# xinntao/EDVR

Measured on AMD Instinct MI355X. Metric: EDVR-L x4 5-frame 720p clips/sec, higher is better.
Workload: dtype fp32 emulated as 2xf16 (hi+lo, 22-bit operands, 4 cross products), fp32 accumulate; 1 GPU; EDVR-L x4, 5 frames, 180x320 LR -> 720x1280, batch 10/GPU, inference; clips_per_gpu=10, global_clips=10, parallelism=clip-sharded x1, no data-path collective, world_size=1, backend=single process

## Files before the change

edvr_amd/_lib.py:

```python
import ctypes
import os

_HERE = os.path.dirname(os.path.abspath(__file__))
LIB_PATH = os.environ.get('EDVR_AMD_LIB') or os.path.join(_HERE, 'lib', 'libedvr_amd.so')

c_float_p = ctypes.c_void_p
i32, i64, f32, sz = ctypes.c_int, ctypes.c_int64, ctypes.c_float, ctypes.c_size_t
vp = ctypes.c_void_p


class ConvDesc(ctypes.Structure):
    _fields_ = [
        ('x1', vp), ('x2', vp), ('c1', i32), ('c2', i32), ('x1_img_stride', i64), ('x2_img_stride', i64),
        ('x2_div', i32), ('x2_mul', i32), ('x2_add', i32), ('n', i32), ('h', i32), ('w', i32), ('wpk', vp),
        ('bias', vp), ('co', i32), ('ks', i32), ('stride', i32), ('act', i32), ('act_from', i32), ('res1', vp),
        ('res2', vp), ('res1_img_stride', i64), ('res2_img_stride', i64), ('y', vp), ('y_img_stride', i64),
        ('out_mode', i32), ('algo', i32), ('gate', vp), ('gate_img_stride', i64), ('gate_slope', f32), ('y_scale', f32),
        ('wpk_f4', vp), ('abs_sum', vp), ('abs_sum_channels', i32), ('wpk_f4s', vp), ('x_amax', vp), ('y_amax', vp),
        ('pre', vp), ('pre_img_stride', i64), ('pre_div', i32), ('pre_mul', i32), ('pre_add', i32), ('pre_n', i32), ('wpk_ds', vp),
    ]


PROTOTYPES = {
    'edvr_version': (ctypes.c_char_p, []),
# ... 14 lines not shown
    'edvr_conv2d_pack_weights_multi': (i32, [vp, i32, i32, i32, vp]),
    'edvr_conv2d_f32': (i32, [ctypes.POINTER(ConvDesc), vp]),
    'edvr_conv2d_kernel': (i32, [ctypes.POINTER(ConvDesc)]),
    'edvr_conv2d_gate_supported': (i32, [ctypes.POINTER(ConvDesc)]),
    'edvr_conv2d_abs_sum_supported': (i32, [ctypes.POINTER(ConvDesc)]),
    'edvr_conv2d_y_amax_supported': (i32, [ctypes.POINTER(ConvDesc)]),
    'edvr_conv2d_pre_supported': (i32, [ctypes.POINTER(ConvDesc)]),
    'edvr_conv2d_f4s_set_lean': (i32, [i32]),
    'edvr_conv2d_f4s_lean_items': (i32, [ctypes.POINTER(ConvDesc)]),
    'edvr_conv2d_kernel_name': (i32, [ctypes.POINTER(ConvDesc), ctypes.c_char_p, sz]),
    'edvr_conv2d_executed_flops': (i32, [ctypes.POINTER(ConvDesc), ctypes.POINTER(ctypes.c_double)]),
    'edvr_dcnv2_fwd_ws_bytes': (sz, [i32] * 12),
    'edvr_dcnv2_fwd_f32': (i32, [vp] * 6 + [i32] * 12 + [i64, i64, i32, i32, vp, sz, vp]),
    'edvr_dcnv2_fwd_split_f32': (i32, [vp] * 6 + [i32] * 12 + [i64, i64, i32, i32, vp, sz, vp, vp]),
    'edvr_dcnv2_fwd_split_applies': (i32, [vp] + [i32] * 13),
    'edvr_dcnv2_fwd_kernel_name': (i32, [vp] + [i32] * 13 + [ctypes.c_char_p, sz]),
    'edvr_dcnv2_bwd_ws_bytes': (sz, [i32] * 12),
    'edvr_dcnv2_any_ws_bytes': (sz, [i32] * 13),
    'edvr_dcnv2_fwd_any': (i32, [i32] + [vp] * 6 + [i32] * 12 + [i64, i64, vp, sz, vp]),
    'edvr_dcnv2_bwd_any': (i32, [i32] + [vp] * 10 + [i32] * 12 + [i64, i64, i64, i64, vp, sz, vp]),
    'edvr_psnr_sse_f32': (i32, [vp, vp, vp, i32, i32, i32, i32, i64, i64, i32, i32, i32, vp]),
    'edvr_ssim_partials': (sz, [i32, i32, i32]),
    'edvr_ssim_f32': (i32, [vp, vp, vp, i32, i32, i32, i32, i64, i64, i32, i32, vp]),
    'edvr_niqe_blocks': (sz, [i32, i32, i32]),
    'edvr_niqe_moments_f32': (i32, [vp, vp, i32, i32, i32, i32, i64, i32, vp]),
    'edvr_niqe_moments_u8': (i32, [vp, vp, i32, i32, i32, i64, i32, vp]),
    'edvr_frames_u8_to_f32': (i32, [vp, vp, i32, i32, i32, i32, vp, i32, vp]),
    'edvr_gather_images_f32': (i32, [vp, vp, vp, vp, i32, vp, i32, i32, vp]),
    'edvr_upsample4x_add_u8': (i32, [vp, vp, vp, i32, i32, i32, vp]),
    'edvr_f32_to_u8_hwc': (i32, [vp, vp, i32, i32, i32, i64, vp]),
# ... 109 lines not shown
```

edvr_amd/csrc/common.h:

```cpp
#pragma once
#include <hip/hip_runtime.h>

#include <cstdarg>
#include <cstdio>

#include "../../include/edvr_amd.h"

namespace edvr {

void set_error(const char *fmt, ...);

inline int check_launch(const char *what) {
  hipError_t e = hipGetLastError();
  if (e != hipSuccess) {
    set_error("%s: %s", what, hipGetErrorString(e));
    return EDVR_ERR_LAUNCH;
  }
  return EDVR_OK;
}

inline hipStream_t as_stream(edvr_stream_t s) { return reinterpret_cast<hipStream_t>(s); }

inline int cdiv(int a, int b) { return (a + b - 1) / b; }
inline int64_t cdiv64(int64_t a, int64_t b) { return (a + b - 1) / b; }
// ... 81 lines not shown
  int64_t doff_bs, dmsk_bs;
};
int dcn_fill_shape(DcnShape &s, int B, int C, int H, int W, int Co, int kh, int kw, int stride, int pad, int dil, int groups, int dg,
                   int64_t off_bs, int64_t msk_bs);

bool dcn_fused_supported(int C, int Co, int H, int W, int kh, int kw, int stride, int pad, int dil, int groups, int dg);
int dcn_fused_pack(const float *weight, float *wpk, int Co, int C, hipStream_t stream);
int dcn_fused_forward(const float *x, const float *offset, const float *mask, const float *wpk, const float *bias, float *y, int B, int C,
                      int H, int W, int Co, int dg, int64_t off_bs, int64_t msk_bs, int act, int halo, hipStream_t stream);

bool dcn_tapwin_supported(int C, int Co, int H, int W, int kh, int kw, int stride, int pad, int dil, int groups, int dg);
int dcn_tapwin_forward(const float *x, const float *offset, const float *mask, const float *wpk, const float *bias, float *y, int B, int C,
                       int H, int W, int Co, int dg, int64_t off_bs, int64_t msk_bs, int act, hipStream_t stream);

bool dcn_tapwin_split_enabled();
int dcn_tapwin_split_forward(const float *x, const float *offset, const float *mask, const float *weight, unsigned *wpk, const float *bias, float *y,
                             int B, int C, int H, int W, int Co, int dg, int64_t off_bs, int64_t msk_bs, int act, const float *xm_amax,
                             hipStream_t stream);

bool dcn_bwd_fused_supported(const DcnShape &s);
size_t dcn_bwd_fused_wbk_elems(int dg);
int dcn_bwd_fused_launch(const DcnShape &s, const float *x, const float *offset, const float *mask, const float *weight, const float *dy,
                         float *wbk, float *col, float *dx, float *doffset, float *dmask, hipStream_t stream);

__device__ inline int xcd_remap(int linear, int total) {
  const int q = total >> 3, rem = total & 7, xcd = linear & 7;
  return xcd * q + (xcd < rem ? xcd : rem) + (linear >> 3);
}
__device__ inline void xcd_block_index(int &bx, int &by, int &bz) {
  const int gx = gridDim.x, gy = gridDim.y;
// ... 17 lines not shown
```

edvr_amd/csrc/dcn.hip:

```cpp
#include <cstdlib>

#include "common.h"
#include "dcn_tap.h"

namespace edvr {

typedef float f32x16 __attribute__((ext_vector_type(16)));

__global__ void fill_kernel(float *__restrict__ p, float v, int64_t n) {
  for (int64_t i = (int64_t)blockIdx.x * blockDim.x + threadIdx.x; i < n; i += (int64_t)gridDim.x * blockDim.x) p[i] = v;
}

struct Merge {
  bool give01, give11;
  bool take00, take10;
};
__device__ __forceinline__ Merge merge_right(const Tap &t, bool same_plane_as_next) {
  Merge mg;
  const int lane = __lane_id();
  const int n_o00 = lane_next_i(t.o00), n_o10 = lane_next_i(t.o10);
  const int n_ok = lane_next_i((t.ok00 ? 1 : 0) | (t.ok10 ? 2 : 0));
  const bool has_next = lane < 63 && same_plane_as_next;
  mg.give01 = has_next && t.ok01 && (n_ok & 1) && n_o00 == t.o01;
  mg.give11 = has_next && t.ok11 && (n_ok & 2) && n_o10 == t.o11;
// ... 653 lines not shown
                             const float *xm_amax, edvr_stream_t stream) {
  EDVR_REQUIRE(xm_amax != nullptr, "dcnv2_fwd_split: null magnitude bound");
  return dcnv2_fwd_impl(x, offset, mask, weight, bias, y, B, C, H, W, Co, kh, kw, stride, pad, dil, groups, dg, offset_bstride, mask_bstride, act,
                        halo_hint, ws, ws_bytes, xm_amax, stream);
}

int edvr_dcnv2_fwd_split_applies(const float *x, int B, int C, int H, int W, int Co, int kh, int kw, int stride, int pad, int dil, int groups,
                                 int dg, int halo_hint) {
  using namespace edvr;
  DcnShape s;
  if (dcn_fill_shape(s, B, C, H, W, Co, kh, kw, stride, pad, dil, groups, dg, 0, 0)) return 0;
  return (use_fused(s) && halo_hint == EDVR_DCN_HALO_TAPWIN && dcn_tapwin_split_enabled() &&
          dcn_tapwin_supported(C, Co, H, W, kh, kw, s.stride, s.pad, s.dil, groups, dg) && (reinterpret_cast<uintptr_t>(x) & 15) == 0) ? 1 : 0;
}

int edvr_dcnv2_fwd_kernel_name(const float *x, int B, int C, int H, int W, int Co, int kh, int kw, int stride, int pad, int dil, int groups,
                               int dg, int halo_hint, char *buf, size_t buf_len) {
  using namespace edvr;
  EDVR_REQUIRE(buf && buf_len > 0, "dcnv2_fwd_kernel_name: null buffer");
  DcnShape s;
  int rc = dcn_fill_shape(s, B, C, H, W, Co, kh, kw, stride, pad, dil, groups, dg, 0, 0);
  if (rc) return rc;
  const char *name = "dcn_im2col_kernel";
  if (use_fused(s) && halo_hint >= 0) {
    const bool tapwin = halo_hint == EDVR_DCN_HALO_TAPWIN && dcn_tapwin_supported(C, Co, H, W, kh, kw, s.stride, s.pad, s.dil, groups, dg) &&
                        (reinterpret_cast<uintptr_t>(x) & 15) == 0;
    name = tapwin ? "dcn_tapwin_fwd_kernel" : "dcn_fused_fwd_kernel";
  }
  snprintf(buf, buf_len, "%s", name);
  return EDVR_OK;
// ... 179 lines not shown
```

edvr_amd/csrc/dcn_tapwin_s.hip:

```cpp
#include <type_traits>

#include "common.h"
#include <cstdlib>

#include "dcn_tap.h"
#include "pack.h"

namespace edvr {

typedef float f32x16 __attribute__((ext_vector_type(16)));
typedef float f32x4 __attribute__((ext_vector_type(4)));
typedef float f32x2 __attribute__((ext_vector_type(2)));

namespace {
constexpr int TWS_TH = 8, TWS_TW = 32, TWS_RY = 2, TWS_RX = 2;
constexpr int TWS_IH = TWS_TH + 2 * TWS_RY;
constexpr int TWS_IW = (TWS_TW + 2 * TWS_RX + 3 + 3) / 4 * 4;
constexpr int TWS_PPR = TWS_IW / 4;
constexpr int TWS_HR = TWS_IH / 2;
constexpr int TWS_HB = TWS_HR * TWS_IW;
constexpr int TWS_CHS = TWS_IH * TWS_IW;
static_assert(TWS_HR * TWS_PPR <= 64 && TWS_IH == 2 * TWS_HR && TWS_CHS % 64 == 32, "window halves must fit one wave instruction");
constexpr int TWS_MAX_DG = 8;
constexpr int TWS_OOB = (int)0x80000000;
// ... 36 lines not shown
  const uint64_t pv = reinterpret_cast<uint64_t>(ptr);
  const uint64_t pu = ((uint64_t)(uint32_t)__builtin_amdgcn_readfirstlane((int)(pv >> 32)) << 32) |
                      (uint32_t)__builtin_amdgcn_readfirstlane((int)(uint32_t)pv);
  return __builtin_amdgcn_make_buffer_rsrc(reinterpret_cast<void *>(pu), (short)0, bytes, TWS_RSRC_FLAGS);
}

static __device__ __forceinline__ void tws_split4(const float (&x)[4], unsigned (&o)[4]) {
  asm volatile(
      "v_fma_mixlo_f16 %0, %4, 1.0, 0\n\tv_fma_mixlo_f16 %1, %5, 1.0, 0\n\tv_fma_mixlo_f16 %2, %6, 1.0, 0\n\tv_fma_mixlo_f16 %3, %7, 1.0, 0\n\t"
      "v_fma_mixhi_f16 %0, %4, 1.0, -%0 op_sel_hi:[0,0,1]\n\tv_fma_mixhi_f16 %1, %5, 1.0, -%1 op_sel_hi:[0,0,1]\n\t"
      "v_fma_mixhi_f16 %2, %6, 1.0, -%2 op_sel_hi:[0,0,1]\n\tv_fma_mixhi_f16 %3, %7, 1.0, -%3 op_sel_hi:[0,0,1]"
      : "=&v"(o[0]), "=&v"(o[1]), "=&v"(o[2]), "=&v"(o[3])
      : "v"(x[0]), "v"(x[1]), "v"(x[2]), "v"(x[3]));
}

template <int MT, int CPG>
__global__ __launch_bounds__(256, 2) void dcn_tapwin_split_fwd_kernel(const DcnTapwinSArgs a) {
  constexpr int TH = TWS_TH, TW = TWS_TW, IH = TWS_IH, IW = TWS_IW, CHS = TWS_CHS, KK = 9, OOB = TWS_OOB;
  constexpr int MB = 32 * MT, NQ = CPG / 2, KG = CPG / 8;
  constexpr int XW = CPG * CHS;
  constexpr int WS = CPG * MB;
  constexpr int CPW = CPG / 4;
  static_assert(CPG % 4 == 0, "four waves share the channels of a group");
  __shared__ __attribute__((aligned(16))) float xw[2 * XW];
  __shared__ __attribute__((aligned(16))) unsigned wsl[2 * WS];
  __shared__ int shifts[TWS_MAX_DG * 18];
  __shared__ float tpl[4 * 3 * 64];

  const int tid = threadIdx.x, lane = tid & 63, half = lane >> 5, j = lane & 31;
  const int wave = __builtin_amdgcn_readfirstlane(tid >> 6);
  const unsigned amax_bits = (unsigned)__builtin_amdgcn_readfirstlane(__builtin_bit_cast(int, *a.xm_amax));
  const float s_x = __builtin_bit_cast(float, (unsigned)min(max(127 + 14 - ((int)((amax_bits >> 23) & 255u) - 127), 7), 220) << 23);
  const float unscale = (1.f / s_x) * __builtin_bit_cast(float, __builtin_amdgcn_readfirstlane((int)a.wpk[1]));
  int tile, blk_y, img;
  xcd_block_index(tile, blk_y, img);
  tile = __builtin_amdgcn_readfirstlane(tile);
  blk_y = __builtin_amdgcn_readfirstlane(blk_y);
  img = __builtin_amdgcn_readfirstlane(img);
  const int ty0 = (tile / a.tiles_x) * TH, tx0 = (tile % a.tiles_x) * TW;
  const int co_blk = a.co_start + blk_y * MB;
  const int P = a.H * a.W;
  const float *x_img = a.x + (int64_t)img * a.C * P;
  const float *off_b = a.offset + (int64_t)img * a.off_bs;
  const float *msk_b = a.mask + (int64_t)img * a.msk_bs;

  for (int v = tid; v < a.dg * 18; v += 256) {
    const float *pl = off_b + (int64_t)v * P;
    float mn = 3.0e38f, mx = -3.0e38f;
#pragma unroll
    for (int r = 1; r < TH; r += 4) {
      const int yy = min(ty0 + r, a.H - 1);
#pragma unroll
      for (int c = 4; c < TW; c += 8) {
        const float f = pl[yy * a.W + min(tx0 + c, a.W - 1)];
        mn = fminf(mn, f);
        mx = fmaxf(mx, f);
      }
    }
    const float mid = fminf(fmaxf(0.5f * (mn + mx), -16384.f), 16384.f);
    shifts[v] = (int)floorf(mid + 0.5f);
  }

  const int oy0 = ty0 + 2 * wave, ox = tx0 + j;
  const bool ok0 = oy0 < a.H && ox < a.W, ok1 = oy0 + 1 < a.H && ox < a.W;
  const int p0 = oy0 * a.W + ox;
  const int tvo[2] = {ok0 ? p0 * 4 : OOB, ok1 ? (p0 + a.W) * 4 : OOB};

  f32x16 acc[2][MT];
#pragma unroll
  for (int s = 0; s < 2; ++s)
#pragma unroll
    for (int m = 0; m < MT; ++m)
#pragma unroll
      for (int r = 0; r < 16; ++r) acc[s][m][r] = 0.f;

  const int d_r = lane / TWS_PPR, d_c = 4 * (lane - d_r * TWS_PPR);
  const int rel0 = (d_r * a.W + d_c) * 4;
  const __amdgpu_buffer_rsrc_t x_rsrc = tws_rsrc(x_img, a.C * P * 4);
  const i32x4 x_rsrc4 = tws_rsrc4(x_img, a.C * P * 4), w_rsrc4 = tws_rsrc4(a.wpk, 64 + a.C * KK * a.cop * 4);
  typedef __attribute__((address_space(3))) void lvoid;
  const unsigned xw_lds = (unsigned)(size_t)(lvoid *)xw, ws_lds = (unsigned)(size_t)(lvoid *)wsl;
  const __amdgpu_buffer_rsrc_t off_rsrc = tws_rsrc(off_b, a.dg * 18 * P * 4), msk_rsrc = tws_rsrc(msk_b, a.dg * 9 * P * 4);
  auto dma_x = [&](int buf, int g, int wy0, int wx0) {
    const int sh = (wy0 * a.W + wx0) * 4;
    const bool colok = (unsigned)(wx0 + d_c) < (unsigned)a.W;
    const int vo0 = (colok && (unsigned)(wy0 + d_r) < (unsigned)a.H) ? rel0 + sh : OOB;
    const int vo1 = (colok && (unsigned)(wy0 + d_r + TWS_HR) < (unsigned)a.H) ? rel0 + sh + TWS_HR * a.W * 4 : OOB;
    if (lane < TWS_HR * TWS_PPR) {
#pragma unroll
      for (int cc = 0; cc < CPW; ++cc) {
        const int ch = wave * CPW + cc;
        const unsigned dst = xw_lds + (buf * XW + ch * CHS) * 4;
        tws_dma16(x_rsrc4, dst, vo0, (g * CPG + ch) * P * 4);
        tws_dma16(x_rsrc4, dst + TWS_HB * 4, vo1, (g * CPG + ch) * P * 4);
      }
    }
  };
  constexpr int WTOTAL = (CPG / 4) * MB, WNI = WTOTAL / 64, WNK = (WNI + 3) / 4;
  static_assert(WTOTAL % 64 == 0, "weight slab must fill whole wave instructions");
  int wvo[WNK];
#pragma unroll
  for (int k = 0; k < WNK; ++k) {
    const int q = (wave + 4 * k) * 64 + lane, row = q / MB, c16 = q - row * MB;
    wvo[k] = (row * KK * a.cop + c16) * 16;
  }
  auto dma_w = [&](int buf, int g, int t) {
    const int so = 64 + ((g * (CPG / 4) * KK + t) * a.cop + co_blk) * 16;
#pragma unroll
    for (int k = 0; k < WNK; ++k)
      if (wave + 4 * k < WNI) tws_dma16(w_rsrc4, ws_lds + (buf * WS + (wave + 4 * k) * 256) * 4, wvo[k], so);
  };
  auto origin = [&](int g, int t, int &wy0, int &wx0) {
    const int sy = __builtin_amdgcn_readfirstlane(shifts[(g * KK + t) * 2]);
    const int sx = __builtin_amdgcn_readfirstlane(shifts[(g * KK + t) * 2 + 1]);
    const int ti = t / 3, tj = t - 3 * ti;
    wy0 = ty0 - 1 + ti + sy - TWS_RY;
    wx0 = (tx0 - 1 + tj + sx - TWS_RX) & ~3;
  };
  const i32x4 off_rsrc4 = tws_rsrc4(off_b, a.dg * 18 * P * 4), msk_rsrc4 = tws_rsrc4(msk_b, a.dg * 9 * P * 4);
  const unsigned tpl_lds = (unsigned)(size_t)(lvoid *)tpl + wave * (3 * 64 * 4);
  const int tvd = half ? tvo[1] : tvo[0];
  auto dma_taps = [&](int g, int t) {
    tws_dma4(off_rsrc4, tpl_lds, tvd, (g * 18 + 2 * t) * P * 4);
    tws_dma4(off_rsrc4, tpl_lds + 256, tvd, (g * 18 + 2 * t + 1) * P * 4);
    tws_dma4(msk_rsrc4, tpl_lds + 512, tvd, (g * 9 + t) * P * 4);
  };
  auto read_taps = [&](float (&d)[6]) {
#pragma unroll
    for (int s = 0; s < 2; ++s)
#pragma unroll
      for (int v = 0; v < 3; ++v) d[3 * s + v] = tpl[wave * 192 + v * 64 + s * 32 + j];
  };

  struct St {
    float bw[2][4];
    int addr[2];
    unsigned slow;
    unsigned slow_any;
  };
  auto state_half = [&](St &st, int s, int t, int wy0, int wx0, const float (&d)[6]) {
    const int ti = t / 3, tj = t - 3 * ti;
    const bool pix_ok = s ? ok1 : ok0;
    const float h = (float)(oy0 + s - 1 + ti) + d[3 * s], w = (float)(ox - 1 + tj) + d[3 * s + 1];
    const bool valid = pix_ok && h > -1.f && w > -1.f && h < (float)a.H && w < (float)a.W;
    const float fh = floorf(h), fw = floorf(w);
    const float lh = h - fh, lw = w - fw, m = d[3 * s + 2];
    const int ry = (int)fh - wy0, rx = (int)fw - wx0;
    const bool inside = valid && ry >= 0 && ry <= IH - 2 && rx >= 0 && rx <= IW - 2;
    const float mm = inside ? m * s_x : 0.f;
    const float hm = (1.f - lh) * mm, lm = lh * mm, hw = 1.f - lw;
    st.bw[s][0] = hm * hw;
    st.bw[s][1] = hm * lw;
    st.bw[s][2] = lm * hw;
    st.bw[s][3] = lm * lw;
    st.addr[s] = half * CHS + (inside ? ry * IW + rx : 0);
    st.slow = (s ? st.slow : 0u) | ((valid && !inside) ? 1u << s : 0u);
  };
  auto state_any = [&](St &st) { st.slow_any = __builtin_amdgcn_readfirstlane(__any(st.slow != 0) ? 1 : 0); };
  auto make_state = [&](St &st, int t, int wy0, int wx0, const float (&d)[6]) {
    state_half(st, 0, t, wy0, wx0, d);
    state_half(st, 1, t, wy0, wx0, d);
    state_any(st);
  };

  auto run_step = [&](auto SLOWT, const St &cur, const float *xb, const unsigned *wb, int g, int t, St &nxt, int tn, int ny0, int nx0,
                      const float (&tnv)[6]) {
    constexpr bool SLOW = decltype(SLOWT)::value;
    const float (&bw)[2][4] = cur.bw;
    const unsigned slow = cur.slow;
    const unsigned cbase[2] = {(unsigned)(size_t)(lvoid *)xb + (unsigned)cur.addr[0] * 4u, (unsigned)(size_t)(lvoid *)xb + (unsigned)cur.addr[1] * 4u};
    auto issue_cells = [&](int kg, float (&c)[2][4][4]) {
#pragma unroll
      for (int s = 0; s < 2; ++s) {
        typedef __attribute__((address_space(3))) const float lds_cf;
        unsigned co = cbase[s];
        asm volatile("" : "+v"(co));
#pragma unroll
        for (int i = 0; i < 4; ++i) {
          lds_cf *cell = (lds_cf *)(size_t)(co + (kg * 8 + 2 * i) * (CHS * 4));
          c[s][i][0] = cell[0];
          c[s][i][1] = cell[1];
          c[s][i][2] = cell[IW];
          c[s][i][3] = cell[IW + 1];
        }
      }
    };
    auto sample = [&](int s, const float (&c)[4]) -> float {
      return __builtin_fmaf(bw[s][3], c[3], __builtin_fmaf(bw[s][2], c[2], __builtin_fmaf(bw[s][1], c[1], bw[s][0] * c[0])));
    };
    if constexpr (SLOW) {
      const int ti = t / 3, tj = t - 3 * ti;
#pragma unroll
      for (int s = 0; s < 2; ++s) {
        if (!__any(slow >> s & 1u)) continue;
        const bool on = slow >> s & 1u;
        const int pv = on ? (p0 + s * a.W) * 4 : OOB;
        const float m = s_x * __builtin_bit_cast(float, __builtin_amdgcn_raw_buffer_load_b32(msk_rsrc, pv, (g * 9 + t) * P * 4, 0));
        const float hsp = (float)(oy0 + s - 1 + ti) + __builtin_bit_cast(float, __builtin_amdgcn_raw_buffer_load_b32(off_rsrc, pv, (g * 18 + 2 * t) * P * 4, 0));
        const float wsp = (float)(ox - 1 + tj) + __builtin_bit_cast(float, __builtin_amdgcn_raw_buffer_load_b32(off_rsrc, pv, (g * 18 + 2 * t + 1) * P * 4, 0));
        const Tap tq = resolve_tap(hsp, wsp, a.H, a.W);
        const float sw[4] = {on ? tq.w00 * m : 0.f, on ? tq.w01 * m : 0.f, on ? tq.w10 * m : 0.f, on ? tq.w11 * m : 0.f};
        const int hp = half * P;
        const int ov[4] = {on ? (tq.o00 + hp) * 4 : OOB, on ? (tq.o01 + hp) * 4 : OOB, on ? (tq.o10 + hp) * 4 : OOB, on ? (tq.o11 + hp) * 4 : OOB};
        float gv[KG][4][4];
#pragma unroll
        for (int kg = 0; kg < KG; ++kg)
#pragma unroll
          for (int i = 0; i < 4; ++i)
#pragma unroll
            for (int c = 0; c < 4; ++c)
              gv[kg][i][c] = __builtin_bit_cast(float, __builtin_amdgcn_raw_buffer_load_b32(x_rsrc, ov[c], (g * CPG + 8 * kg + 2 * i) * P * 4, 0));
#pragma unroll
        for (int kg = 0; kg < KG; ++kg) {
          i32x4 aw[MT];
#pragma unroll
          for (int m2 = 0; m2 < MT; ++m2) aw[m2] = *reinterpret_cast<const i32x4 *>(wb + ((kg * 2 + half) * MB + m2 * 32 + j) * 4);
          float v[4];
#pragma unroll
          for (int i = 0; i < 4; ++i)
            v[i] = __builtin_fmaf(sw[3], gv[kg][i][3], __builtin_fmaf(sw[2], gv[kg][i][2], __builtin_fmaf(sw[1], gv[kg][i][1], sw[0] * gv[kg][i][0])));
          unsigned pk[4];
          tws_split4(v, pk);
          i32x4 bq = i32x4{(int)pk[0], (int)pk[1], (int)pk[2], (int)pk[3]};
#pragma unroll
          for (int m2 = 0; m2 < MT; ++m2)
            acc[s][m2] = __builtin_amdgcn_mfma_f32_32x32x16_f16(__builtin_bit_cast(f16x8, aw[m2]), __builtin_bit_cast(f16x8, bq), acc[s][m2], 0, 0, 0);
          asm volatile("v_alignbit_b32 %0, %0, %0, 16\n\tv_alignbit_b32 %1, %1, %1, 16\n\tv_alignbit_b32 %2, %2, %2, 16\n\tv_alignbit_b32 %3, %3, %3, 16"
                       : "+v"(bq[0]), "+v"(bq[1]), "+v"(bq[2]), "+v"(bq[3]));
#pragma unroll
          for (int m2 = 0; m2 < MT; ++m2)
            acc[s][m2] = __builtin_amdgcn_mfma_f32_32x32x16_f16(__builtin_bit_cast(f16x8, aw[m2]), __builtin_bit_cast(f16x8, bq), acc[s][m2], 0, 0, 0);
        }
      }
    } else {
      float cv[2][4][4];
      issue_cells(0, cv);
#pragma unroll
      for (int kg = 0; kg < KG; ++kg) {
        i32x4 aw[MT];
#pragma unroll
        for (int m = 0; m < MT; ++m) aw[m] = *reinterpret_cast<const i32x4 *>(wb + ((kg * 2 + half) * MB + m * 32 + j) * 4);
        i32x4 bq[2];
#pragma unroll
        for (int s = 0; s < 2; ++s) {
          const float v[4] = {sample(s, cv[s][0]), sample(s, cv[s][1]), sample(s, cv[s][2]), sample(s, cv[s][3])};
          unsigned pk[4];
          tws_split4(v, pk);
          bq[s] = i32x4{(int)pk[0], (int)pk[1], (int)pk[2], (int)pk[3]};
        }
        if (kg + 1 < KG) issue_cells(kg + 1, cv);
#pragma unroll
        for (int s = 0; s < 2; ++s)
#pragma unroll
          for (int m = 0; m < MT; ++m)
            acc[s][m] = __builtin_amdgcn_mfma_f32_32x32x16_f16(__builtin_bit_cast(f16x8, aw[m]), __builtin_bit_cast(f16x8, bq[s]), acc[s][m], 0, 0, 0);
        if (kg == 0 || KG == 1) {
          state_half(nxt, 0, tn, ny0, nx0, tnv);
#pragma unroll
          for (int i = 0; i < 4; ++i) asm volatile("" : "+v"(nxt.bw[0][i]));
          asm volatile("" : "+v"(nxt.addr[0]), "+v"(nxt.slow));
        }
        if (kg == KG - 1) {
          state_half(nxt, 1, tn, ny0, nx0, tnv);
#pragma unroll
          for (int i = 0; i < 4; ++i) asm volatile("" : "+v"(nxt.bw[1][i]));
          asm volatile("" : "+v"(nxt.addr[1]), "+v"(nxt.slow));
          state_any(nxt);
          asm volatile("" : "+s"(nxt.slow_any));
        }
#pragma unroll
        for (int s = 0; s < 2; ++s)
          asm volatile("v_alignbit_b32 %0, %0, %0, 16\n\tv_alignbit_b32 %1, %1, %1, 16\n\tv_alignbit_b32 %2, %2, %2, 16\n\tv_alignbit_b32 %3, %3, %3, 16"
                       : "+v"(bq[s][0]), "+v"(bq[s][1]), "+v"(bq[s][2]), "+v"(bq[s][3]));
#pragma unroll
        for (int s = 0; s < 2; ++s)
#pragma unroll
          for (int m = 0; m < MT; ++m)
            acc[s][m] = __builtin_amdgcn_mfma_f32_32x32x16_f16(__builtin_bit_cast(f16x8, aw[m]), __builtin_bit_cast(f16x8, bq[s]), acc[s][m], 0, 0, 0);
        __builtin_amdgcn_sched_barrier(0);
      }
    }
  };

  __syncthreads();
  const int n_steps = a.dg * KK;
  St cur, nxt;
  float tnv[6];
  int o1y, o1x;
  origin(0, 0, o1y, o1x);
  dma_x(0, 0, o1y, o1x);
  dma_w(0, 0, 0);
  dma_taps(0, 0);
  asm volatile("s_waitcnt vmcnt(0)" ::: "memory");
  read_taps(tnv);
  make_state(cur, 0, o1y, o1x, tnv);
  asm volatile("s_waitcnt lgkmcnt(0)" ::: "memory");
  int g = 0, t = 0, g1 = 0, t1 = 1;
  if (n_steps > 1) {
    origin(g1, t1, o1y, o1x);
    dma_taps(g1, t1);
    asm volatile("s_waitcnt vmcnt(0)" ::: "memory");
  }
// ... 22 lines not shown

  const __amdgpu_buffer_rsrc_t y_rsrc = tws_rsrc(a.y + (int64_t)img * a.Co * P, a.Co * P * 4);
  const __amdgpu_buffer_rsrc_t b_rsrc = tws_rsrc(a.bias ? a.bias : a.x, a.bias ? a.Co * 4 : 0);
#pragma unroll
  for (int m = 0; m < MT; ++m) {
#pragma unroll
    for (int r4 = 0; r4 < 4; ++r4) {
      const int cob = co_blk + m * 32 + 8 * r4;
      float bias4[4];
#pragma unroll
      for (int r = 0; r < 4; ++r) {
        const bool cok = cob + 4 * half + r < a.Co;
        bias4[r] = a.bias ? __builtin_bit_cast(float, __builtin_amdgcn_raw_buffer_load_b32(b_rsrc, cok ? (4 * half + r) * 4 : OOB, cob * 4, 0)) : 0.f;
      }
#pragma unroll
      for (int s = 0; s < 2; ++s) {
        const bool pix_ok = s ? ok1 : ok0;
        const int pv = (p0 + s * a.W + 4 * half * P) * 4;
#pragma unroll
        for (int r = 0; r < 4; ++r) {
          float v = __builtin_fmaf(acc[s][m][4 * r4 + r], unscale, bias4[r]);
          if (a.act == EDVR_ACT_LRELU) v = v > 0.f ? v : 0.1f * v;
          else if (a.act == EDVR_ACT_RELU) v = fmaxf(v, 0.f);
          else if (a.act == EDVR_ACT_SIGMOID) v = __builtin_amdgcn_rcpf(1.f + __expf(-v));
          const bool cok = cob + 4 * half + r < a.Co;
          __builtin_amdgcn_raw_buffer_store_b32(__builtin_bit_cast(unsigned, v), y_rsrc, (pix_ok && cok) ? pv : OOB, (cob + r) * P * 4, 0);
        }
      }
    }
  }
}
// ... 17 lines not shown

__global__ void dcn_tapwin_split_pack_kernel(const float *__restrict__ w, unsigned *__restrict__ wpk, int Co, int C, int cop) {
  const float s_w = __builtin_bit_cast(float, wpk[0]);
  const int64_t total = (int64_t)(C / 4) * 9 * cop;
  const int full = Co / 128, rem_tiles = (Co - full * 128 + 31) / 32;
  for (int64_t i = (int64_t)blockIdx.x * blockDim.x + threadIdx.x; i < total; i += (int64_t)gridDim.x * blockDim.x) {
    const int pos = (int)(i % cop), t = (int)((i / cop) % 9), c4 = (int)(i / ((int64_t)cop * 9));
    const int blk = pos / 128 < full ? pos / 128 : full, start = blk * 128, mt = blk < full ? 4 : rem_tiles;
    const int r = pos - start, co = pos;
    const bool live = mt > 0 && r < 32 * mt && co < Co;
#pragma unroll
    for (int q = 0; q < 4; ++q) wpk[16 + i * 4 + q] = live ? split_f16x2(w[((int64_t)co * C + 8 * (c4 >> 1) + 2 * q + (c4 & 1)) * 9 + t], s_w) : 0u;
  }
}

template <int MT>
static int launch_tapwin_s(DcnTapwinSArgs a, int co_start, int co_blocks, hipStream_t stream) {
  a.co_start = co_start;
  dim3 grid(a.tiles_x * a.tiles_y, co_blocks, a.B);
  if (a.C / a.dg == 16) hipLaunchKernelGGL((dcn_tapwin_split_fwd_kernel<MT, 16>), grid, dim3(256), 0, stream, a);
  else hipLaunchKernelGGL((dcn_tapwin_split_fwd_kernel<MT, 8>), grid, dim3(256), 0, stream, a);
  return check_launch("dcn_tapwin_split_fwd_kernel");
}

bool dcn_tapwin_split_enabled() {
  static const bool on = []() {
    const char *e = getenv("EDVR_DCN_SPLIT");
    return !(e && e[0] == '0');
  }();
  return on;
}

int dcn_tapwin_split_forward(const float *x, const float *offset, const float *mask, const float *weight, unsigned *wpk, const float *bias, float *y,
                             int B, int C, int H, int W, int Co, int dg, int64_t off_bs, int64_t msk_bs, int act, const float *xm_amax,
                             hipStream_t stream) {
  EDVR_REQUIRE(B <= 65535, "dcn_tapwin_split: batch %d exceeds grid.z", B);
// ... 28 lines not shown
```

include/edvr_amd.h:

```cpp
#ifndef EDVR_AMD_H
#define EDVR_AMD_H

#include <stddef.h>
#include <stdint.h>

#ifdef __cplusplus
extern "C" {
#endif

#define EDVR_OK 0
#define EDVR_ERR_ARG (-1)
#define EDVR_ERR_UNSUPPORTED (-2)
#define EDVR_ERR_LAUNCH (-3)
#define EDVR_ERR_WORKSPACE (-4)

typedef void *edvr_stream_t;

const char *edvr_version(void);
const char *edvr_last_error(void);
int edvr_check_device(void);

#define EDVR_ACT_NONE 0
#define EDVR_ACT_RELU 1
#define EDVR_ACT_LRELU 2
// ... 87 lines not shown
#define EDVR_HW(h, w) ((int)(h) | (((int)(w) + 1) << 16))

size_t edvr_dcnv2_fwd_ws_bytes(int B, int C, int H, int W, int Co, int kh, int kw, int stride, int pad, int dil,
                               int groups, int dg);
int edvr_dcnv2_fwd_f32(const float *x, const float *offset, const float *mask, const float *weight,
                       const float *bias, float *y, int B, int C, int H, int W, int Co, int kh, int kw, int stride,
                       int pad, int dil, int groups, int dg, int64_t offset_bstride, int64_t mask_bstride, int act,
                       int halo_hint, void *ws, size_t ws_bytes, edvr_stream_t stream);

int edvr_dcnv2_fwd_split_f32(const float *x, const float *offset, const float *mask, const float *weight, const float *bias,
                             float *y, int B, int C, int H, int W, int Co, int kh, int kw, int stride, int pad, int dil, int groups,
                             int dg, int64_t offset_bstride, int64_t mask_bstride, int act, int halo_hint, void *ws, size_t ws_bytes,
                             const float *xm_amax, edvr_stream_t stream);
int edvr_dcnv2_fwd_split_applies(const float *x, int B, int C, int H, int W, int Co, int kh, int kw, int stride, int pad, int dil, int groups,
                                 int dg, int halo_hint);
int edvr_dcnv2_fwd_kernel_name(const float *x, int B, int C, int H, int W, int Co, int kh, int kw, int stride, int pad, int dil,
                               int groups, int dg, int halo_hint, char *buf, size_t buf_len);

size_t edvr_dcnv2_bwd_ws_bytes(int B, int C, int H, int W, int Co, int kh, int kw, int stride, int pad, int dil,
                               int groups, int dg);
int edvr_dcnv2_bwd_f32(const float *x, const float *offset, const float *mask, const float *weight, const float *dy,
                       float *dx, float *doffset, float *dmask, float *dweight, float *dbias, int B, int C, int H,
                       int W, int Co, int kh, int kw, int stride, int pad, int dil, int groups, int dg,
                       int64_t offset_bstride, int64_t mask_bstride, int64_t doffset_bstride, int64_t dmask_bstride,
                       int scatter_hint, void *ws, size_t ws_bytes, edvr_stream_t stream);
int edvr_dcnv2_bwd_split_f32(const float *x, const float *offset, const float *mask, const float *weight, const float *dy,
                             float *dx, float *doffset, float *dmask, float *dweight, float *dbias, int B, int C, int H,
                             int W, int Co, int kh, int kw, int stride, int pad, int dil, int groups, int dg,
                             int64_t offset_bstride, int64_t mask_bstride, int64_t doffset_bstride, int64_t dmask_bstride,
                             int scatter_hint, void *ws, size_t ws_bytes, const float *xm_amax, const float *dy_amax,
// ... 198 lines not shown
```

Baseline: 106.9 clips/s.

## Add one-row-per-wave variant of split DCN tap-window kernel with 8 waves

Templates the split-precision deformable-conv forward kernel on pixel rows per wave. The new single-row variant launches 512 threads (8 waves) and halves the per-wave accumulators and tap buffers. It is selected by default when channels per group is 16, and an env var or API call can force either mode. The aim is to cut per-wave register pressure and raise wave-level parallelism for better latency hiding. The trade-off is more waves contending for LDS and weight DMA, plus some recomputed lane offsets.

```diff
diff --git a/edvr_amd/_lib.py b/edvr_amd/_lib.py
--- a/edvr_amd/_lib.py
+++ b/edvr_amd/_lib.py
@@ -52,6 +52,7 @@
     'edvr_dcnv2_fwd_f32': (i32, [vp] * 6 + [i32] * 12 + [i64, i64, i32, i32, vp, sz, vp]),
     'edvr_dcnv2_fwd_split_f32': (i32, [vp] * 6 + [i32] * 12 + [i64, i64, i32, i32, vp, sz, vp, vp]),
     'edvr_dcnv2_fwd_split_applies': (i32, [vp] + [i32] * 13),
+    'edvr_dcnv2_fwd_split_set_rows': (i32, [i32]),
     'edvr_dcnv2_fwd_kernel_name': (i32, [vp] + [i32] * 13 + [ctypes.c_char_p, sz]),
     'edvr_dcnv2_bwd_ws_bytes': (sz, [i32] * 12),
     'edvr_dcnv2_any_ws_bytes': (sz, [i32] * 13),
diff --git a/edvr_amd/csrc/common.h b/edvr_amd/csrc/common.h
--- a/edvr_amd/csrc/common.h
+++ b/edvr_amd/csrc/common.h
@@ -119,6 +119,7 @@
                        int H, int W, int Co, int dg, int64_t off_bs, int64_t msk_bs, int act, hipStream_t stream);
 
 bool dcn_tapwin_split_enabled();
+int dcn_tapwin_split_set_rows(int rows);
 int dcn_tapwin_split_forward(const float *x, const float *offset, const float *mask, const float *weight, unsigned *wpk, const float *bias, float *y,
                              int B, int C, int H, int W, int Co, int dg, int64_t off_bs, int64_t msk_bs, int act, const float *xm_amax,
                              hipStream_t stream);
diff --git a/edvr_amd/csrc/dcn.hip b/edvr_amd/csrc/dcn.hip
--- a/edvr_amd/csrc/dcn.hip
+++ b/edvr_amd/csrc/dcn.hip
@@ -691,6 +691,8 @@
           dcn_tapwin_supported(C, Co, H, W, kh, kw, s.stride, s.pad, s.dil, groups, dg) && (reinterpret_cast<uintptr_t>(x) & 15) == 0) ? 1 : 0;
 }
 
+int edvr_dcnv2_fwd_split_set_rows(int rows) { return edvr::dcn_tapwin_split_set_rows(rows); }
+
 int edvr_dcnv2_fwd_kernel_name(const float *x, int B, int C, int H, int W, int Co, int kh, int kw, int stride, int pad, int dil, int groups,
                                int dg, int halo_hint, char *buf, size_t buf_len) {
   using namespace edvr;
diff --git a/edvr_amd/csrc/dcn_tapwin_s.hip b/edvr_amd/csrc/dcn_tapwin_s.hip
--- a/edvr_amd/csrc/dcn_tapwin_s.hip
+++ b/edvr_amd/csrc/dcn_tapwin_s.hip
@@ -1,3 +1,4 @@
+#include <atomic>
 #include <type_traits>
 
 #include "common.h"
@@ -74,18 +75,20 @@
       : "v"(x[0]), "v"(x[1]), "v"(x[2]), "v"(x[3]));
 }
 
-template <int MT, int CPG>
-__global__ __launch_bounds__(256, 2) void dcn_tapwin_split_fwd_kernel(const DcnTapwinSArgs a) {
+template <int MT, int CPG, int SUB>
+__global__ __launch_bounds__(512 / SUB, 4 / SUB) void dcn_tapwin_split_fwd_kernel(const DcnTapwinSArgs a) {
+  static_assert(SUB == 1 || SUB == 2, "one or two pixel rows per wave");
+  constexpr int NW = TWS_TH / SUB;
   constexpr int TH = TWS_TH, TW = TWS_TW, IH = TWS_IH, IW = TWS_IW, CHS = TWS_CHS, KK = 9, OOB = TWS_OOB;
   constexpr int MB = 32 * MT, NQ = CPG / 2, KG = CPG / 8;
   constexpr int XW = CPG * CHS;
   constexpr int WS = CPG * MB;
-  constexpr int CPW = CPG / 4;
-  static_assert(CPG % 4 == 0, "four waves share the channels of a group");
+  constexpr int CPW = CPG / NW;
+  static_assert(CPG % NW == 0, "the waves share the channels of a group");
   __shared__ __attribute__((aligned(16))) float xw[2 * XW];
   __shared__ __attribute__((aligned(16))) unsigned wsl[2 * WS];
   __shared__ int shifts[TWS_MAX_DG * 18];
-  __shared__ float tpl[4 * 3 * 64];
+  __shared__ float tpl[NW * 3 * 32 * SUB];
 
   const int tid = threadIdx.x, lane = tid & 63, half = lane >> 5, j = lane & 31;
   const int wave = __builtin_amdgcn_readfirstlane(tid >> 6);
@@ -104,7 +107,7 @@
   const float *off_b = a.offset + (int64_t)img * a.off_bs;
   const float *msk_b = a.mask + (int64_t)img * a.msk_bs;
 
-  for (int v = tid; v < a.dg * 18; v += 256) {
+  for (int v = tid; v < a.dg * 18; v += 64 * NW) {
     const float *pl = off_b + (int64_t)v * P;
     float mn = 3.0e38f, mx = -3.0e38f;
 #pragma unroll
@@ -121,28 +124,38 @@
     shifts[v] = (int)floorf(mid + 0.5f);
   }
 
-  const int oy0 = ty0 + 2 * wave, ox = tx0 + j;
-  const bool ok0 = oy0 < a.H && ox < a.W, ok1 = oy0 + 1 < a.H && ox < a.W;
+  const int oy0 = ty0 + SUB * wave, ox = tx0 + j;
+  const bool ok0 = oy0 < a.H && ox < a.W, ok1 = SUB == 2 && oy0 + 1 < a.H && ox < a.W;
   const int p0 = oy0 * a.W + ox;
   const int tvo[2] = {ok0 ? p0 * 4 : OOB, ok1 ? (p0 + a.W) * 4 : OOB};
 
-  f32x16 acc[2][MT];
-#pragma unroll
-  for (int s = 0; s < 2; ++s)
+  f32x16 acc[SUB][MT];
+#pragma unroll
+  for (int s = 0; s < SUB; ++s)
 #pragma unroll
     for (int m = 0; m < MT; ++m)
 #pragma unroll
       for (int r = 0; r < 16; ++r) acc[s][m][r] = 0.f;
 
-  const int d_r = lane / TWS_PPR, d_c = 4 * (lane - d_r * TWS_PPR);
-  const int rel0 = (d_r * a.W + d_c) * 4;
+  const int lane_d_r = lane / TWS_PPR, lane_d_c = 4 * (lane - lane_d_r * TWS_PPR);
+  const int lane_rel0 = (lane_d_r * a.W + lane_d_c) * 4;
   const __amdgpu_buffer_rsrc_t x_rsrc = tws_rsrc(x_img, a.C * P * 4);
   const i32x4 x_rsrc4 = tws_rsrc4(x_img, a.C * P * 4), w_rsrc4 = tws_rsrc4(a.wpk, 64 + a.C * KK * a.cop * 4);
   typedef __attribute__((address_space(3))) void lvoid;
   const unsigned xw_lds = (unsigned)(size_t)(lvoid *)xw, ws_lds = (unsigned)(size_t)(lvoid *)wsl;
   const __amdgpu_buffer_rsrc_t off_rsrc = tws_rsrc(off_b, a.dg * 18 * P * 4), msk_rsrc = tws_rsrc(msk_b, a.dg * 9 * P * 4);
+  auto lane_again = [&]() {
+    int l = lane;
+    asm volatile("" : "+v"(l));
+    return l;
+  };
   auto dma_x = [&](int buf, int g, int wy0, int wx0) {
     const int sh = (wy0 * a.W + wx0) * 4;
+    int d_r = lane_d_r, d_c = lane_d_c, rel0 = lane_rel0;
+    if constexpr (SUB == 1) {
+      const int l = lane_again();
+      d_r = l / TWS_PPR, d_c = 4 * (l - d_r * TWS_PPR), rel0 = (d_r * a.W + d_c) * 4;
+    }
     const bool colok = (unsigned)(wx0 + d_c) < (unsigned)a.W;
     const int vo0 = (colok && (unsigned)(wy0 + d_r) < (unsigned)a.H) ? rel0 + sh : OOB;
     const int vo1 = (colok && (unsigned)(wy0 + d_r + TWS_HR) < (unsigned)a.H) ? rel0 + sh + TWS_HR * a.W * 4 : OOB;
@@ -156,19 +169,24 @@
       }
     }
   };
-  constexpr int WTOTAL = (CPG / 4) * MB, WNI = WTOTAL / 64, WNK = (WNI + 3) / 4;
+  constexpr int WTOTAL = (CPG / 4) * MB, WNI = WTOTAL / 64, WNK = (WNI + NW - 1) / NW;
   static_assert(WTOTAL % 64 == 0, "weight slab must fill whole wave instructions");
+  auto w_offset = [&](int k, int l) {
+    const int q = (wave + NW * k) * 64 + l, row = q / MB, c16 = q - row * MB;
+    return (row * KK * a.cop + c16) * 16;
+  };
   int wvo[WNK];
 #pragma unroll
   for (int k = 0; k < WNK; ++k) {
-    const int q = (wave + 4 * k) * 64 + lane, row = q / MB, c16 = q - row * MB;
+    const int q = (wave + NW * k) * 64 + lane, row = q / MB, c16 = q - row * MB;
     wvo[k] = (row * KK * a.cop + c16) * 16;
   }
   auto dma_w = [&](int buf, int g, int t) {
     const int so = 64 + ((g * (CPG / 4) * KK + t) * a.cop + co_blk) * 16;
+    const int l = SUB == 1 ? lane_again() : lane;
 #pragma unroll
     for (int k = 0; k < WNK; ++k)
-      if (wave + 4 * k < WNI) tws_dma16(w_rsrc4, ws_lds + (buf * WS + (wave + 4 * k) * 256) * 4, wvo[k], so);
+      if (wave + NW * k < WNI) tws_dma16(w_rsrc4, ws_lds + (buf * WS + (wave + NW * k) * 256) * 4, SUB == 1 ? w_offset(k, l) : wvo[k], so);
   };
   auto origin = [&](int g, int t, int &wy0, int &wx0) {
     const int sy = __builtin_amdgcn_readfirstlane(shifts[(g * KK + t) * 2]);
@@ -178,27 +196,31 @@
     wx0 = (tx0 - 1 + tj + sx - TWS_RX) & ~3;
   };
   const i32x4 off_rsrc4 = tws_rsrc4(off_b, a.dg * 18 * P * 4), msk_rsrc4 = tws_rsrc4(msk_b, a.dg * 9 * P * 4);
-  const unsigned tpl_lds = (unsigned)(size_t)(lvoid *)tpl + wave * (3 * 64 * 4);
-  const int tvd = half ? tvo[1] : tvo[0];
+  const unsigned tpl_lds = (unsigned)(size_t)(lvoid *)tpl + wave * (3 * 32 * SUB * 4);
+  const int tvd = SUB == 2 ? (half ? tvo[1] : tvo[0]) : ((half && ok0) ? (p0 + P) * 4 : tvo[0]);
   auto dma_taps = [&](int g, int t) {
     tws_dma4(off_rsrc4, tpl_lds, tvd, (g * 18 + 2 * t) * P * 4);
-    tws_dma4(off_rsrc4, tpl_lds + 256, tvd, (g * 18 + 2 * t + 1) * P * 4);
-    tws_dma4(msk_rsrc4, tpl_lds + 512, tvd, (g * 9 + t) * P * 4);
-  };
-  auto read_taps = [&](float (&d)[6]) {
-#pragma unroll
-    for (int s = 0; s < 2; ++s)
-#pragma unroll
-      for (int v = 0; v < 3; ++v) d[3 * s + v] = tpl[wave * 192 + v * 64 + s * 32 + j];
+    if constexpr (SUB == 2) {
+      tws_dma4(off_rsrc4, tpl_lds + 256, tvd, (g * 18 + 2 * t + 1) * P * 4);
+      tws_dma4(msk_rsrc4, tpl_lds + 512, tvd, (g * 9 + t) * P * 4);
+    } else {
+      if (lane < 32) tws_dma4(msk_rsrc4, tpl_lds + 256, tvd, (g * 9 + t) * P * 4);
+    }
+  };
+  auto read_taps = [&](float (&d)[3 * SUB]) {
+#pragma unroll
+    for (int s = 0; s < SUB; ++s)
+#pragma unroll
+      for (int v = 0; v < 3; ++v) d[3 * s + v] = tpl[wave * (96 * SUB) + v * (32 * SUB) + s * 32 + j];
   };
 
   struct St {
-    float bw[2][4];
-    int addr[2];
+    float bw[SUB][4];
+    int addr[SUB];
     unsigned slow;
     unsigned slow_any;
   };
-  auto state_half = [&](St &st, int s, int t, int wy0, int wx0, const float (&d)[6]) {
+  auto state_half = [&](St &st, int s, int t, int wy0, int wx0, const float (&d)[3 * SUB]) {
     const int ti = t / 3, tj = t - 3 * ti;
     const bool pix_ok = s ? ok1 : ok0;
     const float h = (float)(oy0 + s - 1 + ti) + d[3 * s], w = (float)(ox - 1 + tj) + d[3 * s + 1];
@@ -217,21 +239,23 @@
     st.slow = (s ? st.slow : 0u) | ((valid && !inside) ? 1u << s : 0u);
   };
   auto state_any = [&](St &st) { st.slow_any = __builtin_amdgcn_readfirstlane(__any(st.slow != 0) ? 1 : 0); };
-  auto make_state = [&](St &st, int t, int wy0, int wx0, const float (&d)[6]) {
+  auto make_state = [&](St &st, int t, int wy0, int wx0, const float (&d)[3 * SUB]) {
     state_half(st, 0, t, wy0, wx0, d);
-    state_half(st, 1, t, wy0, wx0, d);
+    if constexpr (SUB == 2) state_half(st, 1, t, wy0, wx0, d);
     state_any(st);
   };
 
   auto run_step = [&](auto SLOWT, const St &cur, const float *xb, const unsigned *wb, int g, int t, St &nxt, int tn, int ny0, int nx0,
-                      const float (&tnv)[6]) {
+                      const float (&tnv)[3 * SUB]) {
     constexpr bool SLOW = decltype(SLOWT)::value;
-    const float (&bw)[2][4] = cur.bw;
+    const float (&bw)[SUB][4] = cur.bw;
     const unsigned slow = cur.slow;
-    const unsigned cbase[2] = {(unsigned)(size_t)(lvoid *)xb + (unsigned)cur.addr[0] * 4u, (unsigned)(size_t)(lvoid *)xb + (unsigned)cur.addr[1] * 4u};
-    auto issue_cells = [&](int kg, float (&c)[2][4][4]) {
-#pragma unroll
-      for (int s = 0; s < 2; ++s) {
+    unsigned cbase[SUB];
+#pragma unroll
+    for (int s = 0; s < SUB; ++s) cbase[s] = (unsigned)(size_t)(lvoid *)xb + (unsigned)cur.addr[s] * 4u;
+    auto issue_cells = [&](int kg, float (&c)[SUB][4][4]) {
+#pragma unroll
+      for (int s = 0; s < SUB; ++s) {
         typedef __attribute__((address_space(3))) const float lds_cf;
         unsigned co = cbase[s];
         asm volatile("" : "+v"(co));
@@ -251,7 +275,7 @@
     if constexpr (SLOW) {
       const int ti = t / 3, tj = t - 3 * ti;
 #pragma unroll
-      for (int s = 0; s < 2; ++s) {
+      for (int s = 0; s < SUB; ++s) {
         if (!__any(slow >> s & 1u)) continue;
         const bool on = slow >> s & 1u;
         const int pv = on ? (p0 + s * a.W) * 4 : OOB;
@@ -262,47 +286,82 @@
         const float sw[4] = {on ? tq.w00 * m : 0.f, on ? tq.w01 * m : 0.f, on ? tq.w10 * m : 0.f, on ? tq.w11 * m : 0.f};
         const int hp = half * P;
         const int ov[4] = {on ? (tq.o00 + hp) * 4 : OOB, on ? (tq.o01 + hp) * 4 : OOB, on ? (tq.o10 + hp) * 4 : OOB, on ? (tq.o11 + hp) * 4 : OOB};
-        float gv[KG][4][4];
-#pragma unroll
-        for (int kg = 0; kg < KG; ++kg)
-#pragma unroll
-          for (int i = 0; i < 4; ++i)
-#pragma unroll
-            for (int c = 0; c < 4; ++c)
-              gv[kg][i][c] = __builtin_bit_cast(float, __builtin_amdgcn_raw_buffer_load_b32(x_rsrc, ov[c], (g * CPG + 8 * kg + 2 * i) * P * 4, 0));
-#pragma unroll
-        for (int kg = 0; kg < KG; ++kg) {
-          i32x4 aw[MT];
-#pragma unroll
-          for (int m2 = 0; m2 < MT; ++m2) aw[m2] = *reinterpret_cast<const i32x4 *>(wb + ((kg * 2 + half) * MB + m2 * 32 + j) * 4);
-          float v[4];
-#pragma unroll
-          for (int i = 0; i < 4; ++i)
-            v[i] = __builtin_fmaf(sw[3], gv[kg][i][3], __builtin_fmaf(sw[2], gv[kg][i][2], __builtin_fmaf(sw[1], gv[kg][i][1], sw[0] * gv[kg][i][0])));
-          unsigned pk[4];
-          tws_split4(v, pk);
-          i32x4 bq = i32x4{(int)pk[0], (int)pk[1], (int)pk[2], (int)pk[3]};
-#pragma unroll
-          for (int m2 = 0; m2 < MT; ++m2)
-            acc[s][m2] = __builtin_amdgcn_mfma_f32_32x32x16_f16(__builtin_bit_cast(f16x8, aw[m2]), __builtin_bit_cast(f16x8, bq), acc[s][m2], 0, 0, 0);
-          asm volatile("v_alignbit_b32 %0, %0, %0, 16\n\tv_alignbit_b32 %1, %1, %1, 16\n\tv_alignbit_b32 %2, %2, %2, 16\n\tv_alignbit_b32 %3, %3, %3, 16"
-                       : "+v"(bq[0]), "+v"(bq[1]), "+v"(bq[2]), "+v"(bq[3]));
-#pragma unroll
-          for (int m2 = 0; m2 < MT; ++m2)
-            acc[s][m2] = __builtin_amdgcn_mfma_f32_32x32x16_f16(__builtin_bit_cast(f16x8, aw[m2]), __builtin_bit_cast(f16x8, bq), acc[s][m2], 0, 0, 0);
-        }
+        constexpr int GK = SUB == 2 ? KG : 1;
+#pragma unroll
+        for (int kg0 = 0; kg0 < KG; kg0 += GK) {
+          float gv[GK][4][4];
+#pragma unroll
+          for (int kk = 0; kk < GK; ++kk)
+#pragma unroll
+            for (int i = 0; i < 4; ++i)
+#pragma unroll
+              for (int c = 0; c < 4; ++c)
+                gv[kk][i][c] = __builtin_bit_cast(float, __builtin_amdgcn_raw_buffer_load_b32(x_rsrc, ov[c], (g * CPG + 8 * (kg0 + kk) + 2 * i) * P * 4, 0));
+#pragma unroll
+          for (int kk = 0; kk < GK; ++kk) {
+            const int kg = kg0 + kk;
+            i32x4 aw[MT];
+#pragma unroll
+            for (int m2 = 0; m2 < MT; ++m2) aw[m2] = *reinterpret_cast<const i32x4 *>(wb + ((kg * 2 + half) * MB + m2 * 32 + j) * 4);
+            float v[4];
+#pragma unroll
+            for (int i = 0; i < 4; ++i)
+              v[i] = __builtin_fmaf(sw[3], gv[kk][i][3], __builtin_fmaf(sw[2], gv[kk][i][2], __builtin_fmaf(sw[1], gv[kk][i][1], sw[0] * gv[kk][i][0])));
+            unsigned pk[4];
+            tws_split4(v, pk);
+            i32x4 bq = i32x4{(int)pk[0], (int)pk[1], (int)pk[2], (int)pk[3]};
+#pragma unroll
+            for (int m2 = 0; m2 < MT; ++m2)
+              acc[s][m2] = __builtin_amdgcn_mfma_f32_32x32x16_f16(__builtin_bit_cast(f16x8, aw[m2]), __builtin_bit_cast(f16x8, bq), acc[s][m2], 0, 0, 0);
+            asm volatile("v_alignbit_b32 %0, %0, %0, 16\n\tv_alignbit_b32 %1, %1, %1, 16\n\tv_alignbit_b32 %2, %2, %2, 16\n\tv_alignbit_b32 %3, %3, %3, 16"
+                         : "+v"(bq[0]), "+v"(bq[1]), "+v"(bq[2]), "+v"(bq[3]));
+#pragma unroll
+            for (int m2 = 0; m2 < MT; ++m2)
+              acc[s][m2] = __builtin_amdgcn_mfma_f32_32x32x16_f16(__builtin_bit_cast(f16x8, aw[m2]), __builtin_bit_cast(f16x8, bq), acc[s][m2], 0, 0, 0);
+          }
+        }
+      }
+    } else if constexpr (SUB == 1) {
+#pragma unroll
+      for (int kg = 0; kg < KG; ++kg) {
+        float cv[1][4][4];
+        issue_cells(kg, cv);
+        const float v[4] = {sample(0, cv[0][0]), sample(0, cv[0][1]), sample(0, cv[0][2]), sample(0, cv[0][3])};
+        unsigned pk[4];
+        tws_split4(v, pk);
+        i32x4 bq = i32x4{(int)pk[0], (int)pk[1], (int)pk[2], (int)pk[3]};
+        i32x4 aw[MT];
+#pragma unroll
+        for (int m = 0; m < MT; ++m) aw[m] = *reinterpret_cast<const i32x4 *>(wb + ((kg * 2 + half) * MB + m * 32 + j) * 4);
+#pragma unroll
+        for (int m = 0; m < MT; ++m)
+          acc[0][m] = __builtin_amdgcn_mfma_f32_32x32x16_f16(__builtin_bit_cast(f16x8, aw[m]), __builtin_bit_cast(f16x8, bq), acc[0][m], 0, 0, 0);
+        if (kg == KG - 1) {
+          state_half(nxt, 0, tn, ny0, nx0, tnv);
+#pragma unroll
+          for (int i = 0; i < 4; ++i) asm volatile("" : "+v"(nxt.bw[0][i]));
+          asm volatile("" : "+v"(nxt.addr[0]), "+v"(nxt.slow));
+          state_any(nxt);
+          asm volatile("" : "+s"(nxt.slow_any));
+        }
+        asm volatile("v_alignbit_b32 %0, %0, %0, 16\n\tv_alignbit_b32 %1, %1, %1, 16\n\tv_alignbit_b32 %2, %2, %2, 16\n\tv_alignbit_b32 %3, %3, %3, 16"
+                     : "+v"(bq[0]), "+v"(bq[1]), "+v"(bq[2]), "+v"(bq[3]));
+#pragma unroll
+        for (int m = 0; m < MT; ++m)
+          acc[0][m] = __builtin_amdgcn_mfma_f32_32x32x16_f16(__builtin_bit_cast(f16x8, aw[m]), __builtin_bit_cast(f16x8, bq), acc[0][m], 0, 0, 0);
+        __builtin_amdgcn_sched_barrier(0);
       }
     } else {
-      float cv[2][4][4];
+      float cv[SUB][4][4];
       issue_cells(0, cv);
 #pragma unroll
       for (int kg = 0; kg < KG; ++kg) {
         i32x4 aw[MT];
 #pragma unroll
         for (int m = 0; m < MT; ++m) aw[m] = *reinterpret_cast<const i32x4 *>(wb + ((kg * 2 + half) * MB + m * 32 + j) * 4);
-        i32x4 bq[2];
-#pragma unroll
-        for (int s = 0; s < 2; ++s) {
+        i32x4 bq[SUB];
+#pragma unroll
+        for (int s = 0; s < SUB; ++s) {
           const float v[4] = {sample(s, cv[s][0]), sample(s, cv[s][1]), sample(s, cv[s][2]), sample(s, cv[s][3])};
           unsigned pk[4];
           tws_split4(v, pk);
@@ -310,7 +369,7 @@
         }
         if (kg + 1 < KG) issue_cells(kg + 1, cv);
 #pragma unroll
-        for (int s = 0; s < 2; ++s)
+        for (int s = 0; s < SUB; ++s)
 #pragma unroll
           for (int m = 0; m < MT; ++m)
             acc[s][m] = __builtin_amdgcn_mfma_f32_32x32x16_f16(__builtin_bit_cast(f16x8, aw[m]), __builtin_bit_cast(f16x8, bq[s]), acc[s][m], 0, 0, 0);
@@ -321,19 +380,21 @@
           asm volatile("" : "+v"(nxt.addr[0]), "+v"(nxt.slow));
         }
         if (kg == KG - 1) {
-          state_half(nxt, 1, tn, ny0, nx0, tnv);
-#pragma unroll
-          for (int i = 0; i < 4; ++i) asm volatile("" : "+v"(nxt.bw[1][i]));
-          asm volatile("" : "+v"(nxt.addr[1]), "+v"(nxt.slow));
+          if constexpr (SUB == 2) {
+            state_half(nxt, 1, tn, ny0, nx0, tnv);
+#pragma unroll
+            for (int i = 0; i < 4; ++i) asm volatile("" : "+v"(nxt.bw[1][i]));
+            asm volatile("" : "+v"(nxt.addr[1]), "+v"(nxt.slow));
+          }
           state_any(nxt);
           asm volatile("" : "+s"(nxt.slow_any));
         }
 #pragma unroll
-        for (int s = 0; s < 2; ++s)
+        for (int s = 0; s < SUB; ++s)
           asm volatile("v_alignbit_b32 %0, %0, %0, 16\n\tv_alignbit_b32 %1, %1, %1, 16\n\tv_alignbit_b32 %2, %2, %2, 16\n\tv_alignbit_b32 %3, %3, %3, 16"
                        : "+v"(bq[s][0]), "+v"(bq[s][1]), "+v"(bq[s][2]), "+v"(bq[s][3]));
 #pragma unroll
-        for (int s = 0; s < 2; ++s)
+        for (int s = 0; s < SUB; ++s)
 #pragma unroll
           for (int m = 0; m < MT; ++m)
             acc[s][m] = __builtin_amdgcn_mfma_f32_32x32x16_f16(__builtin_bit_cast(f16x8, aw[m]), __builtin_bit_cast(f16x8, bq[s]), acc[s][m], 0, 0, 0);
@@ -345,7 +406,7 @@
   __syncthreads();
   const int n_steps = a.dg * KK;
   St cur, nxt;
-  float tnv[6];
+  float tnv[3 * SUB];
   int o1y, o1x;
   origin(0, 0, o1y, o1x);
   dma_x(0, 0, o1y, o1x);
@@ -398,7 +459,7 @@
         bias4[r] = a.bias ? __builtin_bit_cast(float, __builtin_amdgcn_raw_buffer_load_b32(b_rsrc, cok ? (4 * half + r) * 4 : OOB, cob * 4, 0)) : 0.f;
       }
 #pragma unroll
-      for (int s = 0; s < 2; ++s) {
+      for (int s = 0; s < SUB; ++s) {
         const bool pix_ok = s ? ok1 : ok0;
         const int pv = (p0 + s * a.W + 4 * half * P) * 4;
 #pragma unroll
@@ -446,12 +507,33 @@
   }
 }
 
+static std::atomic<int> &tapwin_s_rows_switch() {
+  static std::atomic<int> rows([]() {
+    const char *e = getenv("EDVR_DCN_SPLIT_ROWS");
+    return (e && e[0] == '2') ? 2 : (e && e[0] == '1') ? 1 : 0;
+  }());
+  return rows;
+}
+
+int dcn_tapwin_split_set_rows(int rows) { return tapwin_s_rows_switch().exchange(rows == 2 ? 2 : rows == 1 ? 1 : 0); }
+
+static int tapwin_s_rows(const DcnTapwinSArgs &a) {
+  const int asked = tapwin_s_rows_switch().load(std::memory_order_relaxed);
+  return asked ? asked : (a.C / a.dg == 16 ? 1 : 2);
+}
+
 template <int MT>
 static int launch_tapwin_s(DcnTapwinSArgs a, int co_start, int co_blocks, hipStream_t stream) {
   a.co_start = co_start;
   dim3 grid(a.tiles_x * a.tiles_y, co_blocks, a.B);
-  if (a.C / a.dg == 16) hipLaunchKernelGGL((dcn_tapwin_split_fwd_kernel<MT, 16>), grid, dim3(256), 0, stream, a);
-  else hipLaunchKernelGGL((dcn_tapwin_split_fwd_kernel<MT, 8>), grid, dim3(256), 0, stream, a);
+  const bool cpg16 = a.C / a.dg == 16;
+  if (tapwin_s_rows(a) == 1) {
+    if (cpg16) hipLaunchKernelGGL((dcn_tapwin_split_fwd_kernel<MT, 16, 1>), grid, dim3(512), 0, stream, a);
+    else hipLaunchKernelGGL((dcn_tapwin_split_fwd_kernel<MT, 8, 1>), grid, dim3(512), 0, stream, a);
+  } else {
+    if (cpg16) hipLaunchKernelGGL((dcn_tapwin_split_fwd_kernel<MT, 16, 2>), grid, dim3(256), 0, stream, a);
+    else hipLaunchKernelGGL((dcn_tapwin_split_fwd_kernel<MT, 8, 2>), grid, dim3(256), 0, stream, a);
+  }
   return check_launch("dcn_tapwin_split_fwd_kernel");
 }
 
diff --git a/include/edvr_amd.h b/include/edvr_amd.h
--- a/include/edvr_amd.h
+++ b/include/edvr_amd.h
@@ -125,6 +125,7 @@
                              const float *xm_amax, edvr_stream_t stream);
 int edvr_dcnv2_fwd_split_applies(const float *x, int B, int C, int H, int W, int Co, int kh, int kw, int stride, int pad, int dil, int groups,
                                  int dg, int halo_hint);
+int edvr_dcnv2_fwd_split_set_rows(int rows);
 int edvr_dcnv2_fwd_kernel_name(const float *x, int B, int C, int H, int W, int Co, int kh, int kw, int stride, int pad, int dil,
                                int groups, int dg, int halo_hint, char *buf, size_t buf_len);
 
```

New measurement: 107.2 clips/s, median of 6. About the same (+0.3%).
